# MDIL-SNU/SevenNet

Measured on AMD Instinct MI355X. Metric: atom-steps/sec (energy+forces), SevenNet-0 100k-atom cell, 1/2/4/8 MI355X, higher is better.
Workload: dtype f32 (storage / accumulate / tensor product; in-kernel W2 products f16x3 = two fp16 terms per operand, three matrix-core products: fp32-rounding class; node linears bf16x6); 1 GPU; sevennet_0 shape (5 interaction layers), 97336-atom periodic diamond-Si cell (a=5.431 A x 23^3, sigma=0.05 A), cutoff 5.0 A, 2725408 directed edges, seeded synthetic weights; atoms=97336, edges=2725408, parallelism=single GPU, fused=auto, terms=4

## Files before the change

### include/snet_hip.h

```cpp
#ifndef SNET_HIP_H
#define SNET_HIP_H

#include <stdint.h>

#ifdef __cplusplus
extern "C" {
#endif

#define SNET_ABI_VERSION 4

int snet_abi_version(void);
const char *snet_last_error(void);
int snet_conv_num_shapes(void);
const char *snet_conv_shape_tag(int i);

typedef struct snet_edge_params {
  float cutoff;
  int32_t n_basis;
  int32_t cutoff_kind;
  int32_t poly_p;
  float cutoff_on;
  int32_t lmax;
  int32_t normalize;
} snet_edge_params;
// ... 32 lines not shown
  int64_t c_off;
  int32_t n_src, d, N, reserved;
} snet_gemm_multi_desc;
int snet_gemm_multi(const snet_gemm_multi_desc *descs_host, int32_t n_desc, float *C, int64_t n_nodes, int64_t c_node_stride,
                    const int32_t *row_idx, const float *table, const int32_t *types, void *stream);
int64_t snet_gemm_split_size(int32_t K, int32_t N);
int snet_gemm_split_pack(const float *B_host, int32_t K, int32_t N, void *packed_host);
typedef struct snet_mlp_plan snet_mlp_plan;
int snet_radial_mlp_plan_create(int32_t nb, int32_t h1, int32_t h2, int32_t wn, const float *W0_host,
                                const float *W1_host, const float *W2_host, int32_t act, float cst, int32_t mode,
                                snet_mlp_plan **plan);
void snet_radial_mlp_plan_destroy(snet_mlp_plan *plan);
int snet_radial_mlp_fwd(const snet_mlp_plan *plan, const float *emb, int64_t n_edges, float *w_out, void *stream);
int snet_radial_mlp_bwd(const snet_mlp_plan *plan, const float *emb, const float *g_w, int64_t n_edges,
                        float *g_emb, void *stream);

int snet_act_fwd(const float *z, float *a, int64_t n, int32_t act, float cst, void *stream);
int snet_act_bwd(const float *z, const float *g_a, float *g_z, int64_t n, int32_t act, float cst, void *stream);

typedef struct snet_conv_plan snet_conv_plan;
int snet_conv_plan_create(const char *tag, snet_conv_plan **plan);
void snet_conv_plan_destroy(snet_conv_plan *plan);
int snet_conv_register_library(const char *path);
int snet_conv_plan_dims(const snet_conv_plan *plan, int32_t *dx, int32_t *dout, int32_t *nsh, int32_t *wn);

int snet_conv_fwd(const snet_conv_plan *plan, const float *x, const float *sh, const float *w, const int32_t *w_row,
                  const int32_t *row_ptr, const int32_t *src, int64_t n_dst, float scale, float *out,
                  void *stream);
#define SNET_FUSED_TERMS_DEFAULT 4
typedef struct snet_fused_plan snet_fused_plan;
int snet_radial_mlp_hidden_fwd(const snet_mlp_plan *plan, const float *emb, int64_t n_edges, float *h2, void *stream);
int snet_radial_mlp_hidden_fwd_layers(const snet_mlp_plan *const *plans, int32_t n_layers, const float *emb, int64_t n_edges,
                                      float *const *h2, void *stream);
int snet_radial_mlp_hidden_bwd(const snet_mlp_plan *plan, const float *emb, const float *g_h2, int64_t n_edges,
                               float *g_emb, void *stream);
int snet_conv_fused_available(const snet_conv_plan *plan);
int snet_fused_plan_create(const snet_conv_plan *plan, const snet_mlp_plan *mlp, int32_t terms, snet_fused_plan **out);
void snet_fused_plan_destroy(snet_fused_plan *plan);
int snet_edge_tiles(const int32_t *row_ptr, int64_t n_dst, int32_t *tile_ptr, int32_t *tile_node, int64_t tile_capacity,
                    int64_t *n_tiles, void *stream);
int snet_edge_tiles_packed(const int32_t *row_ptr, int64_t node_begin, int64_t node_end, int32_t *tile_e0,
                           int32_t *tile_nodes, int64_t tile_capacity, int64_t *n_tiles, void *stream);
int snet_fused_plan_tile_mode(const snet_fused_plan *plan);
int snet_conv_plan_transposed(const snet_conv_plan *plan, char *tag, float *col_scale, int32_t *dead, int32_t dead_capacity,
                              int32_t *n_dead);
int snet_edges_by_source(const int32_t *row_ptr, int64_t n_dst, const int32_t *eperm, const int32_t *w_row, int64_t n_edges,
                         int32_t *center_t, int32_t *w_row_t, void *stream);
int snet_conv_fwd_fused(const snet_fused_plan *plan, const float *x, const float *sh, const float *h2,
                        const int32_t *w_row, const int32_t *row_ptr, const int32_t *src, int64_t n_dst, float scale,
                        float *out, void *stream);
int snet_conv_bwd_fused(const snet_fused_plan *plan, const float *x, const float *sh, const float *dsh,
                        const float *h2, const int32_t *w_row, const int32_t *row_ptr, const int32_t *src,
                        const int32_t *tile_ptr, const int32_t *tile_node, int64_t n_tiles, float scale,
                        const float *g_out, float *g_xe, float *g_h2, const float *emb, float *g_emb, float *g_vec,
                        const float *x_rowmax, const float *g_rowmax, void *stream);
int snet_conv_bwd_fused_sh(const snet_fused_plan *plan, const float *x, const float *sh, const float *h2, const int32_t *w_row,
                           const int32_t *row_ptr, const int32_t *src, const int32_t *tile_ptr, const int32_t *tile_node,
                           int64_t n_tiles, float scale, const float *g_out, float *g_xe, float *g_h2, const float *emb,
                           float *g_emb, float *g_sh, const float *x_rowmax, const float *g_rowmax, void *stream);
int snet_fused_plan_has_mlp_tail(const snet_fused_plan *plan);
int snet_fused_plan_prefers_tangent(const snet_fused_plan *plan);
int snet_edge_embed_tangent(const snet_edge_params *p_host, const float *coeffs_host, const float *edge_vec,
                            const int32_t *edge_of_row, int64_t n_rows, float *demb, void *stream);
int snet_radial_mlp_hidden_fwd_layers_tangent(const snet_mlp_plan *const *plans, int32_t n_layers, const float *emb, const float *demb,
                                              int64_t n_rows, float *const *h2, float *const *h2d, void *stream);
int snet_conv_bwd_fused_tangent(const snet_fused_plan *plan, const float *x, const float *sh, const float *dsh, const float *h2,
// ... 269 lines not shown
```

### sevennet_amd/_lib.py

```python
from __future__ import annotations

import ctypes as C
import os

_HERE = os.path.dirname(os.path.abspath(__file__))
ABI_VERSION = 4
LIB_PATH = os.environ.get('SNET_HIP_LIB') or os.path.join(_HERE, 'libsnet_hip.so')

c_f32p = C.c_void_p
c_i32p = C.c_void_p
c_f64p = C.c_void_p
c_stream = C.c_void_p


class EdgeParams(C.Structure):
    _fields_ = [('cutoff', C.c_float), ('n_basis', C.c_int32), ('cutoff_kind', C.c_int32),
                ('poly_p', C.c_int32), ('cutoff_on', C.c_float), ('lmax', C.c_int32),
                ('normalize', C.c_int32)]


class GemmDesc(C.Structure):
    _fields_ = [('B', C.c_void_p), ('B_split', C.c_void_p), ('a_off', C.c_int64), ('c_off', C.c_int64), ('d', C.c_int32), ('K', C.c_int32),
                ('N', C.c_int32), ('accumulate', C.c_int32)]

# ... 19 lines not shown
    'snet_conv_num_shapes': (C.c_int, []),
    'snet_conv_shape_tag': (C.c_char_p, [C.c_int]),
    'snet_edge_embed_fwd': (C.c_int, [C.POINTER(EdgeParams), C.POINTER(C.c_float), c_f32p, C.c_int64, c_f32p,
                                      c_f32p, c_f32p, c_stream]),
    'snet_edge_embed_bwd': (C.c_int, [C.POINTER(EdgeParams), C.POINTER(C.c_float), c_f32p, C.c_int64, c_f32p,
                                      c_f32p, c_f32p, C.c_int32, c_stream]),
    'snet_radial_mlp_plan_create': (C.c_int, [C.c_int32, C.c_int32, C.c_int32, C.c_int32, C.POINTER(C.c_float),
                                              C.POINTER(C.c_float), C.POINTER(C.c_float), C.c_int32, C.c_float,
                                              C.c_int32, C.POINTER(C.c_void_p)]),
    'snet_radial_mlp_plan_destroy': (None, [C.c_void_p]),
    'snet_radial_mlp_fwd': (C.c_int, [C.c_void_p, c_f32p, C.c_int64, c_f32p, c_stream]),
    'snet_radial_mlp_bwd': (C.c_int, [C.c_void_p, c_f32p, c_f32p, C.c_int64, c_f32p, c_stream]),
    'snet_conv_bwd_edge_vec': (C.c_int, [C.c_void_p, c_f32p, c_f32p, c_f32p, c_f32p, c_i32p, c_i32p, c_i32p, C.c_int64,
                                         C.c_float, c_f32p, c_f32p, c_f32p, c_f32p, c_stream]),
    'snet_gemm': (C.c_int, [c_f32p, c_f32p, c_f32p, C.c_int64, C.c_int32, C.c_int32, C.c_int32, C.c_int64,
                            C.c_int64, C.c_int64, C.c_int64, c_i32p, C.c_int32, c_stream]),
    'snet_gemm_grouped': (C.c_int, [C.POINTER(GemmDesc), C.c_int32, c_f32p, c_f32p, C.c_int64, C.c_int64, C.c_int64,
                                    c_i32p, c_stream]),
    'snet_gemm_multi': (C.c_int, [C.POINTER(GemmMultiDesc), C.c_int32, c_f32p, C.c_int64, C.c_int64, c_i32p, c_f32p, c_i32p,
                                  c_stream]),
    'snet_gemm_split_size': (C.c_int64, [C.c_int32, C.c_int32]),
    'snet_gemm_split_pack': (C.c_int, [C.c_void_p, C.c_int32, C.c_int32, C.c_void_p]),
    'snet_act_fwd': (C.c_int, [c_f32p, c_f32p, C.c_int64, C.c_int32, C.c_float, c_stream]),
    'snet_act_bwd': (C.c_int, [c_f32p, c_f32p, c_f32p, C.c_int64, C.c_int32, C.c_float, c_stream]),
    'snet_conv_plan_create': (C.c_int, [C.c_char_p, C.POINTER(C.c_void_p)]),
    'snet_conv_plan_destroy': (None, [C.c_void_p]),
    'snet_conv_register_library': (C.c_int, [C.c_char_p]),
    'snet_conv_plan_dims': (C.c_int, [C.c_void_p, C.POINTER(C.c_int32), C.POINTER(C.c_int32),
                                      C.POINTER(C.c_int32), C.POINTER(C.c_int32)]),
    'snet_conv_fwd': (C.c_int, [C.c_void_p, c_f32p, c_f32p, c_f32p, c_i32p, c_i32p, c_i32p, C.c_int64, C.c_float,
                                c_f32p, c_stream]),
    'snet_radial_mlp_hidden_fwd': (C.c_int, [C.c_void_p, c_f32p, C.c_int64, c_f32p, c_stream]),
    'snet_radial_mlp_hidden_fwd_layers': (C.c_int, [C.POINTER(C.c_void_p), C.c_int32, c_f32p, C.c_int64, C.POINTER(C.c_void_p), c_stream]),
    'snet_radial_mlp_hidden_bwd': (C.c_int, [C.c_void_p, c_f32p, c_f32p, C.c_int64, c_f32p, c_stream]),
    'snet_conv_fused_available': (C.c_int, [C.c_void_p]),
    'snet_conv_plan_transposed': (C.c_int, [C.c_void_p, C.c_char_p, c_f32p, c_i32p, C.c_int32, C.POINTER(C.c_int32)]),
    'snet_edges_by_source': (C.c_int, [c_i32p, C.c_int64, c_i32p, c_i32p, C.c_int64, c_i32p, c_i32p, c_stream]),
    'snet_fused_plan_create': (C.c_int, [C.c_void_p, C.c_void_p, C.c_int32, C.POINTER(C.c_void_p)]),
    'snet_fused_plan_destroy': (None, [C.c_void_p]),
    'snet_edge_tiles': (C.c_int, [c_i32p, C.c_int64, c_i32p, c_i32p, C.c_int64, C.POINTER(C.c_int64), c_stream]),
    'snet_conv_fwd_fused': (C.c_int, [C.c_void_p, c_f32p, c_f32p, c_f32p, c_i32p, c_i32p, c_i32p, C.c_int64, C.c_float,
                                      c_f32p, c_stream]),
    'snet_conv_bwd_fused': (C.c_int, [C.c_void_p, c_f32p, c_f32p, c_f32p, c_f32p, c_i32p, c_i32p, c_i32p, c_i32p,
                                      c_i32p, C.c_int64, C.c_float, c_f32p, c_f32p, c_f32p, c_f32p, c_f32p, c_f32p, c_f32p, c_f32p,
                                      c_stream]),
    'snet_conv_bwd_fused_sh': (C.c_int, [C.c_void_p, c_f32p, c_f32p, c_f32p, c_i32p, c_i32p, c_i32p, c_i32p,
                                         c_i32p, C.c_int64, C.c_float, c_f32p, c_f32p, c_f32p, c_f32p, c_f32p, c_f32p, c_f32p, c_f32p,
                                         c_stream]),
    'snet_fused_plan_has_mlp_tail': (C.c_int, [C.c_void_p]),
    'snet_fused_plan_prefers_tangent': (C.c_int, [C.c_void_p]),
    'snet_edge_embed_tangent': (C.c_int, [C.POINTER(EdgeParams), C.POINTER(C.c_float), c_f32p, c_i32p, C.c_int64, c_f32p, c_stream]),
    'snet_radial_mlp_hidden_fwd_layers_tangent': (C.c_int, [C.POINTER(C.c_void_p), C.c_int32, c_f32p, c_f32p, C.c_int64,
                                                            C.POINTER(C.c_void_p), C.POINTER(C.c_void_p), c_stream]),
    'snet_conv_bwd_fused_tangent': (C.c_int, [C.c_void_p, c_f32p, c_f32p, c_f32p, c_f32p, c_f32p, c_i32p, c_i32p, c_i32p, c_i32p,
                                              c_i32p, C.c_int64, C.c_float, c_f32p, c_f32p, c_f32p, c_f32p, c_f32p, c_f32p,
                                              c_stream]),
    'snet_model_set_layer0_moments': (C.c_int, [C.c_void_p, C.c_int32]),
    'snet_layer0_plan_create': (C.c_int, [C.c_void_p, C.c_void_p, C.c_void_p, C.c_float, C.c_int32, C.POINTER(C.c_void_p)]),
    'snet_layer0_fold': (C.c_int, [C.c_void_p, C.c_int32, C.c_int32, C.c_void_p, C.c_float, C.c_int32, C.c_int32, C.c_void_p]),
    'snet_layer0_plan_destroy': (None, [C.c_void_p]),
    'snet_layer0_scratch_size': (C.c_int64, [C.c_void_p, C.c_int64]),
    'snet_layer0_conv_bwd': (C.c_int, [C.c_void_p, c_f32p, c_f32p, c_f32p, c_i32p, c_i32p, c_i32p, c_i32p, c_i32p, c_f32p, c_f32p, c_f32p,
                                       C.c_int64, c_f32p, c_f32p, c_stream]),
    'snet_model_set_last_layer_merged': (C.c_int, [C.c_void_p, C.c_int32]),
    'snet_lastlayer_plan_create': (C.c_int, [C.c_void_p, C.c_void_p, C.POINTER(C.c_void_p)]),
    'snet_lastlayer_plan_destroy': (None, [C.c_void_p]),
# ... 198 lines not shown
```

### sevennet_amd/csrc/snet_mlp.hip

```cpp
#include <algorithm>
#include <cmath>
#include <cstring>
#include <initializer_list>
#include <vector>

#include "snet_common.h"
#include "snet_split.h"

namespace {

using namespace snet;
constexpr int H = 64;

__device__ __forceinline__ int krow(int s, int half) { return 32 * (s >> 4) + (s & 3) + 8 * ((s & 15) >> 2) + 4 * half; }

__device__ __forceinline__ void hidden_forward(const float *__restrict__ emb, int64_t e_lane, bool e_ok, int nb,
                                               const float *__restrict__ W0, const float *W1s, int act, float cst,
                                               int lane, f32x16 (&z1)[2], f32x16 (&a1)[2], f32x16 (&z2)[2]) {
  const int half = lane >> 5, li = lane & 31;
  z1[0] = zero16();
  z1[1] = zero16();
  for (int s = 0; 2 * s < nb; ++s) {
    const int k = 2 * s + half;
    const float b = (e_ok && k < nb) ? emb[e_lane * nb + k] : 0.f;
// ... 328 lines not shown
    if (more) {
#pragma unroll
      for (int i = 0; i < 3; ++i) st[i] = W2B[(int64_t)(c + 1) * W2B_TILE_U4 + tid + 256 * i];
    }
    f32x16 acc = zero16();
#pragma unroll
    for (int q = 0; q < 4; ++q) {
      bf16x8 b[3];
#pragma unroll
      for (int t = 0; t < 3; ++t) b[t] = as_bf16x8(slab[buf][(q * 3 + t) * 64 + lane]);
      acc = mfma6(a2[q], b, acc);
    }
    const int ch = 32 * c + li;
    if (wave_ok && ch < wn) {
#pragma unroll
      for (int r = 0; r < 16; ++r) {
        const int64_t e = e0 + (r & 3) + 8 * (r >> 2) + 4 * half;
        if (e < E) w_out[e * wn + ch] = acc[r];
      }
    }
    if (more) {
#pragma unroll
      for (int i = 0; i < 3; ++i) slab[buf ^ 1][tid + 256 * i] = st[i];
    }
    __syncthreads();
    buf ^= 1;
  }
}

constexpr int MAX_HIDDEN_LAYERS = 8;
struct HiddenLayers {
  const float *W0[MAX_HIDDEN_LAYERS];
  const u32x4 *W1A[MAX_HIDDEN_LAYERS];
  float *h2[MAX_HIDDEN_LAYERS];
  float *h2d[MAX_HIDDEN_LAYERS];
  float cst[MAX_HIDDEN_LAYERS];
  int act[MAX_HIDDEN_LAYERS];
  int n;
};

template <int ACT, int NB>
__global__ __launch_bounds__(256, 2) void radial_mlp_hidden_layers_kernel(const float *__restrict__ emb, int64_t E, int nb,
                                                                       HiddenLayers P) {
  const int tid = threadIdx.x;
  const int lane = tid & 63, wave = __builtin_amdgcn_readfirstlane(tid >> 6);
  const int half = lane >> 5, li = lane & 31;
  const int64_t e_lane = ((int64_t)blockIdx.x * 4 + wave) * 32 + li;
  const bool e_ok = e_lane < E;
  for (int l = 0; l < P.n; ++l) {
    const int act = P.act[l];
    const float cst = P.cst[l];
    f32x16 z1[2], z2[2];
    hidden_forward_split<ACT, NB>(emb, e_ok ? e_lane : 0, e_ok, nb, P.W0[l], P.W1A[l], act, cst, lane, z1, z2);
    if (!e_ok) continue;
    float *__restrict__ h2 = P.h2[l];
#pragma unroll
    for (int t = 0; t < 2; ++t)
#pragma unroll
      for (int g = 0; g < 4; ++g) {
        f32x4 v;
#pragma unroll
        for (int i = 0; i < 4; ++i) v[i] = act_sel<ACT>(z2[t][4 * g + i], act) * cst;
        *reinterpret_cast<f32x4 *>(h2 + e_lane * H + 32 * t + 8 * g + 4 * half) = v;
      }
  }
}

template <int ACT>
__device__ __forceinline__ void act_pair_sel(float z, int act, float &f, float &g) {
  if constexpr (ACT >= 0) snet::act_pair_radial(z, ACT, f, g);
  else snet::act_pair_radial(z, act, f, g);
}

template <int ACT, int NB>
__global__ __launch_bounds__(256, 2) void radial_mlp_hidden_layers_tangent_kernel(const float *__restrict__ emb,
                                                                               const float *__restrict__ demb, int64_t E, int nb,
                                                                               HiddenLayers P) {
  const int tid = threadIdx.x;
  const int lane = tid & 63, wave = __builtin_amdgcn_readfirstlane(tid >> 6);
  const int half = lane >> 5, li = lane & 31;
  const int64_t e_raw = ((int64_t)blockIdx.x * 4 + wave) * 32 + li;
  const bool e_ok = e_raw < E;
  const int64_t e_lane = e_ok ? e_raw : 0;
  for (int l = 0; l < P.n; ++l) {
    const int act = P.act[l];
    const float cst = P.cst[l];
    const float *__restrict__ W0 = P.W0[l];
    const u32x4 *__restrict__ W1A = P.W1A[l];
    f32x16 z1[2], z1d[2], z2[2], z2d[2];
#pragma unroll
    for (int t = 0; t < 2; ++t) z1[t] = z1d[t] = z2[t] = z2d[t] = zero16();
    auto l1_step = [&](int s, int n_basis) {
      const int k = 2 * s + half;
      const float b = (e_ok && k < n_basis) ? emb[e_lane * n_basis + k] : 0.f;
      const float bd = (e_ok && k < n_basis) ? demb[e_lane * n_basis + k] : 0.f;
#pragma unroll
      for (int t = 0; t < 2; ++t) {
        const float a = (k < n_basis) ? W0[k * H + 32 * t + li] : 0.f;
        z1[t] = __builtin_amdgcn_mfma_f32_32x32x2f32(a, b, z1[t], 0, 0, 0);
        z1d[t] = __builtin_amdgcn_mfma_f32_32x32x2f32(a, bd, z1d[t], 0, 0, 0);
      }
    };
    if constexpr (NB > 0) {
#pragma unroll
      for (int s = 0; 2 * s < NB; ++s) l1_step(s, NB);
    } else {
      for (int s = 0; 2 * s < nb; ++s) l1_step(s, nb);
    }
#pragma unroll
    for (int q = 0; q < 4; ++q) {
      float v[8], vd[8];
#pragma unroll
      for (int i = 0; i < 8; ++i) {
        float f, g;
        act_pair_sel<ACT>(z1[q >> 1][8 * (q & 1) + i], act, f, g);
        v[i] = f * cst;
        vd[i] = g * cst * z1d[q >> 1][8 * (q & 1) + i];
      }
      const Split3 b = split8(v), bd = split8(vd);
#pragma unroll
      for (int to = 0; to < 2; ++to) {
        bf16x8 a[3];
        load_frag3(W1A, to * 4 + q, lane, a);
        z2[to] = mfma6(a, b, z2[to]);
        z2d[to] = mfma6(a, bd, z2d[to]);
      }
    }
    if (!e_ok) continue;
    float *__restrict__ h2 = P.h2[l];
    float *__restrict__ h2d = P.h2d[l];
#pragma unroll
    for (int t = 0; t < 2; ++t)
#pragma unroll
      for (int g = 0; g < 4; ++g) {
        f32x4 v, vd;
#pragma unroll
        for (int i = 0; i < 4; ++i) {
          float f, d;
          act_pair_sel<ACT>(z2[t][4 * g + i], act, f, d);
          v[i] = f * cst;
          vd[i] = d * cst * z2d[t][4 * g + i];
        }
        *reinterpret_cast<f32x4 *>(h2 + e_lane * H + 32 * t + 8 * g + 4 * half) = v;
        *reinterpret_cast<f32x4 *>(h2d + e_lane * H + 32 * t + 8 * g + 4 * half) = vd;
      }
  }
}

#ifndef SNET_MLP_BWD_OCC
#define SNET_MLP_BWD_OCC 3
#endif
#ifndef SNET_MLP_BWD_WAVES
#define SNET_MLP_BWD_WAVES 4
#endif
constexpr int GS_STRIDE = 36;
constexpr int GS_TILE = 32 * GS_STRIDE;
constexpr int SLAB_U4 = 2 * 2 * 3 * 64;

__global__ __launch_bounds__(64 * SNET_MLP_BWD_WAVES, SNET_MLP_BWD_OCC) void radial_mlp_bwd_split_kernel(
    const float *__restrict__ emb, const float *__restrict__ g_w, int64_t E, int nb, int wn,
    const float *__restrict__ W0, const u32x4 *__restrict__ W1A, const u32x4 *__restrict__ W2A,
    const u32x4 *__restrict__ W1A2, const u32x4 *__restrict__ W0A, int act, float cst, float *__restrict__ g_emb) {
  constexpr int NWV = SNET_MLP_BWD_WAVES, NTH = 64 * NWV, NSL = (768 + NTH - 1) / NTH;
  __shared__ float gws[NWV * GS_TILE];
  __shared__ u32x4 slab[2][SLAB_U4];
  const int tid = threadIdx.x;
  const int lane = tid & 63, wave = __builtin_amdgcn_readfirstlane(tid >> 6);
  const int half = lane >> 5, li = lane & 31;
  const int64_t e0 = ((int64_t)blockIdx.x * NWV + wave) * 32;
  const bool wave_ok = e0 < E;
  const int64_t e_lane = e0 + li;
  const bool e_ok = wave_ok && e_lane < E;
  float *tile = gws + wave * GS_TILE;
  const bool vec_ok = (wn & 3) == 0;
  const int srow = lane >> 3, scol = 4 * (lane & 7);
  const int n_chunks = (wn + CH - 1) / CH;

  f32x4 st_g[2][4];
  u32x4 st_w[2][NSL];
// ... 147 lines not shown
      ga1[to] = mfma6(a, b, ga1[to]);
    }
  }
  f32x16 ge = zero16();
#pragma unroll
  for (int q = 0; q < 4; ++q) {
    float v[8];
#pragma unroll
    for (int i = 0; i < 8; ++i) {
      const int r = 8 * (q & 1) + i;
      v[i] = ga1[q >> 1][r] * cst * snet::act_grad(z1[q >> 1][r], act);
    }
    const Split3 b = split8(v);
    bf16x8 a[3];
    load_frag3(W0A, q, lane, a);
    ge = mfma6(a, b, ge);
  }
  if (e_ok) {
#pragma unroll
    for (int r = 0; r < 16; ++r) {
      const int k0 = (r & 3) + 8 * (r >> 2) + 4 * half;
      if (k0 < nb) g_emb[e_lane * nb + k0] += ge[r];
    }
  }
}

}

struct snet_mlp_plan {
  int nb, wn, act, mode;
  float cst;
  float *W0 = nullptr, *W1 = nullptr, *W2 = nullptr, *W2T = nullptr;
  u32x4 *W1A = nullptr, *W2B = nullptr, *W2A = nullptr, *W1A2 = nullptr, *W0A = nullptr;
  std::vector<float> w2_host;
  std::vector<float> w0_host, w1_host;
};

namespace {

inline uint16_t bf16_rne(float v) {
  uint32_t u;
  memcpy(&u, &v, 4);
  u += 0x7fffu + ((u >> 16) & 1u);
  return (uint16_t)(u >> 16);
}
inline float bf16_f(uint16_t h) {
  const uint32_t u = (uint32_t)h << 16;
  float f;
  memcpy(&f, &u, 4);
  return f;
}
inline void split3(float x, uint16_t (&o)[3]) {
  o[0] = bf16_rne(x);
  const float r1 = x - bf16_f(o[0]);
  o[1] = bf16_rne(r1);
  o[2] = bf16_rne(r1 - bf16_f(o[1]));
}
inline int kmap(int q, int half, int i8) {
  const int r = 8 * (q & 1) + i8;
  return 32 * (q >> 1) + (r & 3) + 8 * (r >> 2) + 4 * half;
}
template <class F>
std::vector<uint16_t> pack_frags(int n_frag, F value) {
  std::vector<uint16_t> out((size_t)n_frag * 3 * 64 * 8);
  for (int f = 0; f < n_frag; ++f)
    for (int lane = 0; lane < 64; ++lane)
      for (int i = 0; i < 8; ++i) {
        uint16_t s[3];
        split3(value(f, lane, i), s);
        for (int t = 0; t < 3; ++t) out[(((size_t)f * 3 + t) * 64 + lane) * 8 + i] = s[t];
      }
  return out;
}
template <class T>
int upload(const std::vector<T> &h, void **dev) {
  if (hipMalloc(dev, h.size() * sizeof(T)) != hipSuccess) return 1;
  return hipMemcpy(*dev, h.data(), h.size() * sizeof(T), hipMemcpyHostToDevice) != hipSuccess;
}

}

extern "C" int snet_radial_mlp_plan_create(int32_t nb, int32_t h1, int32_t h2, int32_t wn, const float *W0_host,
                                           const float *W1_host, const float *W2_host, int32_t act, float cst,
                                           int32_t mode, snet_mlp_plan **plan) {
  SNET_REQUIRE(plan != nullptr && W0_host && W1_host && W2_host, "snet_radial_mlp_plan_create: null argument");
  SNET_REQUIRE(h1 == H && h2 == H, "snet_radial_mlp_plan_create: fused kernels need hidden widths [64, 64]");
  SNET_REQUIRE(nb >= 1 && nb <= 32 && wn >= 1, "snet_radial_mlp_plan_create: need 1 <= n_basis <= 32, wn >= 1");
  SNET_REQUIRE(act >= 0 && act < snet::N_ACT, "snet_radial_mlp_plan_create: unknown activation");
  SNET_REQUIRE(mode == 0 || mode == 1, "snet_radial_mlp_plan_create: mode 0 (fp32 MFMA) or 1 (bf16 x6 split)");
  auto *p = new snet_mlp_plan;
  p->nb = nb; p->wn = wn; p->act = act; p->mode = mode; p->cst = cst;
  const std::vector<float> w0(W0_host, W0_host + (size_t)nb * H), w1(W1_host, W1_host + (size_t)H * H),
      w2(W2_host, W2_host + (size_t)H * wn);
  int bad = upload(w0, (void **)&p->W0);
  if (mode == 0) {
    std::vector<float> w2t((size_t)wn * H);
    for (int k = 0; k < H; ++k)
      for (int c = 0; c < wn; ++c) w2t[(size_t)c * H + k] = w2[(size_t)k * wn + c];
    bad |= upload(w1, (void **)&p->W1) | upload(w2, (void **)&p->W2) | upload(w2t, (void **)&p->W2T);
  } else {
    const int n_tiles = (wn + 31) / 32, n_chunks = (wn + CH - 1) / CH;
    bad |= upload(pack_frags(8, [&](int f, int lane, int i) {
                    const int to = f >> 2, q = f & 3;
                    return w1[(size_t)kmap(q, lane >> 5, i) * H + 32 * to + (lane & 31)];
                  }), (void **)&p->W1A);
    bad |= upload(pack_frags(n_tiles * 4, [&](int f, int lane, int i) {
                    const int c = f >> 2, q = f & 3, ch = 32 * c + (lane & 31);
                    return ch < wn ? w2[(size_t)kmap(q, lane >> 5, i) * wn + ch] : 0.f;
                  }), (void **)&p->W2B);
    bad |= upload(pack_frags(n_chunks * 4, [&](int f, int lane, int i) {
                    const int t = f & 1, s = (f >> 1) & 1, ck = f >> 2;
                    const int ch = ck * CH + 16 * s + 8 * (lane >> 5) + i;
                    return ch < wn ? w2[(size_t)(32 * t + (lane & 31)) * wn + ch] : 0.f;
                  }), (void **)&p->W2A);
    bad |= upload(pack_frags(8, [&](int f, int lane, int i) {
                    const int to = f >> 2, q = f & 3;
                    return w1[(size_t)(32 * to + (lane & 31)) * H + kmap(q, lane >> 5, i)];
                  }), (void **)&p->W1A2);
    bad |= upload(pack_frags(4, [&](int f, int lane, int i) {
                    const int k0 = lane & 31;
                    return k0 < nb ? w0[(size_t)k0 * H + kmap(f, lane >> 5, i)] : 0.f;
                  }), (void **)&p->W0A);
  }
  p->w2_host = w2;
  p->w0_host = w0;
  p->w1_host = w1;
  if (bad) {
    snet::set_error("snet_radial_mlp_plan_create: device allocation / upload failed");
    delete p;
    return 1;
  }
  *plan = p;
  return 0;
}

extern "C" void snet_radial_mlp_plan_destroy(snet_mlp_plan *p) {
  if (!p) return;
  for (void *d : {(void *)p->W0, (void *)p->W1, (void *)p->W2, (void *)p->W2T, (void *)p->W1A, (void *)p->W2B,
                  (void *)p->W2A, (void *)p->W1A2, (void *)p->W0A})
    if (d) (void)hipFree(d);
  delete p;
}

extern "C" int snet_radial_mlp_fwd(const snet_mlp_plan *p, const float *emb, int64_t E, float *w_out, void *stream) {
  SNET_REQUIRE(p != nullptr, "snet_radial_mlp_fwd: null plan");
  if (E <= 0) return 0;
  const int64_t grid = (E + 127) / 128;
  SNET_REQUIRE(grid < (1ll << 31), "snet_radial_mlp_fwd: too many edges");
  hipStream_t st = static_cast<hipStream_t>(stream);
  if (p->mode == 0)
    radial_mlp_fwd_kernel<<<(unsigned)grid, 256, 0, st>>>(emb, E, p->nb, p->wn, p->W0, p->W1, p->W2, p->act, p->cst,
                                                          w_out);
  else
    radial_mlp_fwd_split_kernel<<<(unsigned)grid, 256, 0, st>>>(emb, E, p->nb, p->wn, p->W0, p->W1A, p->W2B, p->act,
                                                                p->cst, w_out);
  SNET_CHECK_LAUNCH("snet_radial_mlp_fwd");
  return 0;
}

extern "C" int snet_radial_mlp_hidden_fwd_layers(const snet_mlp_plan *const *plans, int32_t n_layers, const float *emb, int64_t E,
                                                 float *const *h2, void *stream) {
  SNET_REQUIRE(plans != nullptr && h2 != nullptr, "snet_radial_mlp_hidden_fwd_layers: null argument");
  SNET_REQUIRE(n_layers >= 1 && n_layers <= MAX_HIDDEN_LAYERS, "snet_radial_mlp_hidden_fwd_layers: 1 .. 8 layers per call");
  HiddenLayers P{};
  P.n = n_layers;
  bool silu = true;
  for (int l = 0; l < n_layers; ++l) {
    const snet_mlp_plan *p = plans[l];
    SNET_REQUIRE(p != nullptr, "snet_radial_mlp_hidden_fwd_layers: null plan");
    SNET_REQUIRE(E <= 0 || h2[l] != nullptr, "snet_radial_mlp_hidden_fwd_layers: null output");
    SNET_REQUIRE(p->mode == 1, "snet_radial_mlp_hidden_fwd_layers: split-precision plans only (mode 1)");
    SNET_REQUIRE(p->nb == plans[0]->nb, "snet_radial_mlp_hidden_fwd_layers: the layers must share the edge embedding (same n_basis)");
    P.W0[l] = p->W0; P.W1A[l] = p->W1A; P.h2[l] = h2[l]; P.cst[l] = p->cst; P.act[l] = p->act;
    silu = silu && p->act == 0;
  }
  if (E <= 0) return 0;
  const int64_t grid = (E + 127) / 128;
  SNET_REQUIRE(grid < (1ll << 31), "snet_radial_mlp_hidden_fwd_layers: too many edges");
  hipStream_t st = static_cast<hipStream_t>(stream);
  const int nb = plans[0]->nb;
  if (silu && nb == 8) radial_mlp_hidden_layers_kernel<0, 8><<<(unsigned)grid, 256, 0, st>>>(emb, E, nb, P);
  else if (silu) radial_mlp_hidden_layers_kernel<0, 0><<<(unsigned)grid, 256, 0, st>>>(emb, E, nb, P);
  else radial_mlp_hidden_layers_kernel<-1, 0><<<(unsigned)grid, 256, 0, st>>>(emb, E, nb, P);
  SNET_CHECK_LAUNCH("snet_radial_mlp_hidden_fwd_layers");
  return 0;
}

extern "C" int snet_radial_mlp_hidden_fwd_layers_tangent(const snet_mlp_plan *const *plans, int32_t n_layers, const float *emb,
                                                         const float *demb, int64_t E, float *const *h2, float *const *h2d, void *stream) {
  SNET_REQUIRE(plans != nullptr && h2 != nullptr && h2d != nullptr, "snet_radial_mlp_hidden_fwd_layers_tangent: null argument");
  SNET_REQUIRE(n_layers >= 1 && n_layers <= MAX_HIDDEN_LAYERS, "snet_radial_mlp_hidden_fwd_layers_tangent: 1 .. 8 layers per call");
  HiddenLayers P{};
  P.n = n_layers;
  bool silu = true;
  for (int l = 0; l < n_layers; ++l) {
    const snet_mlp_plan *p = plans[l];
    SNET_REQUIRE(p != nullptr, "snet_radial_mlp_hidden_fwd_layers_tangent: null plan");
    SNET_REQUIRE(E <= 0 || (h2[l] != nullptr && h2d[l] != nullptr), "snet_radial_mlp_hidden_fwd_layers_tangent: null output");
    SNET_REQUIRE(p->mode == 1, "snet_radial_mlp_hidden_fwd_layers_tangent: split-precision plans only (mode 1)");
    SNET_REQUIRE(p->nb == plans[0]->nb, "snet_radial_mlp_hidden_fwd_layers_tangent: the layers must share the edge embedding (same n_basis)");
    P.W0[l] = p->W0; P.W1A[l] = p->W1A; P.h2[l] = h2[l]; P.h2d[l] = h2d[l]; P.cst[l] = p->cst; P.act[l] = p->act;
    silu = silu && p->act == 0;
  }
  if (E <= 0) return 0;
  SNET_REQUIRE(emb != nullptr && demb != nullptr, "snet_radial_mlp_hidden_fwd_layers_tangent: null input");
  const int64_t grid = (E + 127) / 128;
  SNET_REQUIRE(grid < (1ll << 31), "snet_radial_mlp_hidden_fwd_layers_tangent: too many edges");
  hipStream_t st = static_cast<hipStream_t>(stream);
  const int nb = plans[0]->nb;
  if (silu && nb == 8) radial_mlp_hidden_layers_tangent_kernel<0, 8><<<(unsigned)grid, 256, 0, st>>>(emb, demb, E, nb, P);
  else if (silu) radial_mlp_hidden_layers_tangent_kernel<0, 0><<<(unsigned)grid, 256, 0, st>>>(emb, demb, E, nb, P);
  else radial_mlp_hidden_layers_tangent_kernel<-1, 0><<<(unsigned)grid, 256, 0, st>>>(emb, demb, E, nb, P);
  SNET_CHECK_LAUNCH("snet_radial_mlp_hidden_fwd_layers_tangent");
  return 0;
}

extern "C" int snet_radial_mlp_hidden_fwd(const snet_mlp_plan *p, const float *emb, int64_t E, float *h2, void *stream) {
  SNET_REQUIRE(p != nullptr, "snet_radial_mlp_hidden_fwd: null plan");
  return snet_radial_mlp_hidden_fwd_layers(&p, 1, emb, E, &h2, stream);
}

namespace snet {
int mlp_plan_wn(const snet_mlp_plan *plan) { return plan ? plan->wn : 0; }
const float *mlp_plan_w2_host(const snet_mlp_plan *plan) {
  return (plan && !plan->w2_host.empty()) ? plan->w2_host.data() : nullptr;
}

MlpHidden mlp_plan_hidden(const snet_mlp_plan *plan) {
  MlpHidden h{nullptr, nullptr, 0, 0, 0.f};
  if (plan && plan->mode == 1 && !plan->w0_host.empty())
    h = MlpHidden{plan->w0_host.data(), plan->w1_host.data(), plan->nb, plan->act, plan->cst};
  return h;
}
uint16_t f16_rne(float f) {
  uint32_t u;
  std::memcpy(&u, &f, 4);
  const uint16_t sign = (uint16_t)((u >> 16) & 0x8000u);
  const uint32_t a = u & 0x7fffffffu;
  if (a >= 0x7f800000u) return sign | (a > 0x7f800000u ? 0x7e00u : 0x7c00u);
  if (a >= 0x477ff000u) return sign | 0x7c00u;
  if (a < 0x33000001u) return sign;
  if (a < 0x38800000u) {
    const int shift = 126 - (int)(a >> 23);
    const uint32_t m = (a & 0x7fffffu) | 0x800000u;
    const uint32_t q = m >> shift, rem = m & ((1u << shift) - 1), half = 1u << (shift - 1);
    return sign | (uint16_t)(q + ((rem > half || (rem == half && (q & 1))) ? 1 : 0));
  }
  const uint32_t r = a + 0xfffu + ((a >> 13) & 1);
  return sign | (uint16_t)((r - 0x38000000u) >> 13);
}
float f16_f(uint16_t h) {
  const uint32_t sign = (uint32_t)(h & 0x8000u) << 16, e = (h >> 10) & 31, m = h & 0x3ffu;
// ... 126 lines not shown
```

Before: 2.857 million atom-steps/s.

## Stage hidden MLP outputs through LDS tiles and keep L1 inputs in registers

Merges the plain and tangent hidden-layer kernels into one templated body. The body loads the edge embedding once, prefetches the next layer's W0 into registers, and applies activations over whole accumulator tiles. Output rows of h2/h2d are staged through a per-wave swizzled LDS tile so global stores are full contiguous 256-byte rows instead of strided 16-byte pieces. An optional scaled two-term f16 matrix-core path for W1 is added behind a compile flag that is off by default. The cost is extra LDS and wave barriers, plus possible register pressure from holding the L1 operands.

```diff
diff --git a/include/snet_hip.h b/include/snet_hip.h
--- a/include/snet_hip.h
+++ b/include/snet_hip.h
@@ -88,6 +88,7 @@
 int snet_radial_mlp_hidden_fwd(const snet_mlp_plan *plan, const float *emb, int64_t n_edges, float *h2, void *stream);
 int snet_radial_mlp_hidden_fwd_layers(const snet_mlp_plan *const *plans, int32_t n_layers, const float *emb, int64_t n_edges,
                                       float *const *h2, void *stream);
+int snet_radial_mlp_pack_w1_f16(const float *W1_host, uint16_t *frags, int32_t *exp_out);
 int snet_radial_mlp_hidden_bwd(const snet_mlp_plan *plan, const float *emb, const float *g_h2, int64_t n_edges,
                                float *g_emb, void *stream);
 int snet_conv_fused_available(const snet_conv_plan *plan);
diff --git a/sevennet_amd/_lib.py b/sevennet_amd/_lib.py
--- a/sevennet_amd/_lib.py
+++ b/sevennet_amd/_lib.py
@@ -75,6 +75,7 @@
                                 c_f32p, c_stream]),
     'snet_radial_mlp_hidden_fwd': (C.c_int, [C.c_void_p, c_f32p, C.c_int64, c_f32p, c_stream]),
     'snet_radial_mlp_hidden_fwd_layers': (C.c_int, [C.POINTER(C.c_void_p), C.c_int32, c_f32p, C.c_int64, C.POINTER(C.c_void_p), c_stream]),
+    'snet_radial_mlp_pack_w1_f16': (C.c_int, [C.POINTER(C.c_float), C.c_void_p, C.POINTER(C.c_int32)]),
     'snet_radial_mlp_hidden_bwd': (C.c_int, [C.c_void_p, c_f32p, c_f32p, C.c_int64, c_f32p, c_stream]),
     'snet_conv_fused_available': (C.c_int, [C.c_void_p]),
     'snet_conv_plan_transposed': (C.c_int, [C.c_void_p, C.c_char_p, c_f32p, c_i32p, C.c_int32, C.POINTER(C.c_int32)]),
diff --git a/sevennet_amd/csrc/snet_mlp.hip b/sevennet_amd/csrc/snet_mlp.hip
--- a/sevennet_amd/csrc/snet_mlp.hip
+++ b/sevennet_amd/csrc/snet_mlp.hip
@@ -384,39 +384,195 @@
 struct HiddenLayers {
   const float *W0[MAX_HIDDEN_LAYERS];
   const u32x4 *W1A[MAX_HIDDEN_LAYERS];
+  const u32x4 *W1H[MAX_HIDDEN_LAYERS];
   float *h2[MAX_HIDDEN_LAYERS];
   float *h2d[MAX_HIDDEN_LAYERS];
   float cst[MAX_HIDDEN_LAYERS];
   int act[MAX_HIDDEN_LAYERS];
+  int w1_exp[MAX_HIDDEN_LAYERS];
   int n;
 };
 
-template <int ACT, int NB>
-__global__ __launch_bounds__(256, 2) void radial_mlp_hidden_layers_kernel(const float *__restrict__ emb, int64_t E, int nb,
-                                                                       HiddenLayers P) {
-  const int tid = threadIdx.x;
-  const int lane = tid & 63, wave = __builtin_amdgcn_readfirstlane(tid >> 6);
+#ifndef SNET_HIDDEN_F16
+#define SNET_HIDDEN_F16 0
+#endif
+#ifndef SNET_HIDDEN_OCC
+#define SNET_HIDDEN_OCC 2
+#endif
+
+__device__ __forceinline__ f32x16 mfma32_f16(bf16x8 a, bf16x8 b, f32x16 acc) {
+  return __builtin_amdgcn_mfma_f32_32x32x16_f16(__builtin_bit_cast(f16x8, a), __builtin_bit_cast(f16x8, b), acc, 0, 0, 0);
+}
+
+__device__ __forceinline__ int tile_scale_exp(const f32x16 (&a)[2]) {
+  float m = 0.f;
+#pragma unroll
+  for (int t = 0; t < 2; ++t)
+#pragma unroll
+    for (int r = 0; r < 16; ++r) m = fmaxf(m, fabsf(a[t][r]));
+  return min(60, F16_TOP - bound_exp(wave_max(m)));
+}
+
+template <int ACT, bool TANGENT>
+__device__ __forceinline__ void hidden_l2(const f32x16 (&a)[2], const f32x16 (&ad)[2], const u32x4 *__restrict__ W1A,
+                                          const u32x4 *__restrict__ W1H, int w1_exp, int lane, f32x16 (&z2)[2], f32x16 (&z2d)[2]) {
+#pragma unroll
+  for (int t = 0; t < 2; ++t) z2[t] = z2d[t] = zero16();
+  if constexpr (ACT >= 0 && SNET_HIDDEN_F16) {
+    u32x4 w[2][2][2];
+    auto load_w = [&](int q) {
+#pragma unroll
+      for (int to = 0; to < 2; ++to)
+#pragma unroll
+        for (int term = 0; term < 2; ++term) w[q & 1][to][term] = W1H[((to * 4 + q) * 2 + term) * 64 + lane];
+    };
+    load_w(0);
+    const int k = tile_scale_exp(a);
+    int kd = 0;
+    if constexpr (TANGENT) kd = tile_scale_exp(ad);
+    const float up = pow2f(k), upd = pow2f(kd);
+#pragma unroll
+    for (int q = 0; q < 4; ++q) {
+      if (q + 1 < 4) {
+        load_w(q + 1);
+        __builtin_amdgcn_sched_barrier(0);
+      }
+      float v[8], vd[8];
+#pragma unroll
+      for (int i = 0; i < 8; ++i) {
+        v[i] = a[q >> 1][8 * (q & 1) + i] * up;
+        if constexpr (TANGENT) vd[i] = ad[q >> 1][8 * (q & 1) + i] * upd;
+      }
+      const SplitN<2> b = splitn8<2, true>(v);
+      SplitN<2> bd;
+      if constexpr (TANGENT) bd = splitn8<2, true>(vd);
+#pragma unroll
+      for (int to = 0; to < 2; ++to) {
+        const bf16x8 w_hi = as_bf16x8(w[q & 1][to][0]), w_lo = as_bf16x8(w[q & 1][to][1]);
+        z2[to] = mfma32_f16(w_hi, b.t[1], z2[to]);
+        z2[to] = mfma32_f16(w_lo, b.t[0], z2[to]);
+        z2[to] = mfma32_f16(w_hi, b.t[0], z2[to]);
+        if constexpr (TANGENT) {
+          z2d[to] = mfma32_f16(w_hi, bd.t[1], z2d[to]);
+          z2d[to] = mfma32_f16(w_lo, bd.t[0], z2d[to]);
+          z2d[to] = mfma32_f16(w_hi, bd.t[0], z2d[to]);
+        }
+      }
+    }
+    const float down = pow2f(-(k + w1_exp)), downd = pow2f(-(kd + w1_exp));
+#pragma unroll
+    for (int t = 0; t < 2; ++t)
+#pragma unroll
+      for (int r = 0; r < 16; ++r) {
+        z2[t][r] *= down;
+        if constexpr (TANGENT) z2d[t][r] *= downd;
+      }
+  } else {
+#pragma unroll
+    for (int q = 0; q < 4; ++q) {
+      float v[8], vd[8];
+#pragma unroll
+      for (int i = 0; i < 8; ++i) {
+        v[i] = a[q >> 1][8 * (q & 1) + i];
+        if constexpr (TANGENT) vd[i] = ad[q >> 1][8 * (q & 1) + i];
+      }
+      const Split3 b = split8(v);
+      Split3 bd;
+      if constexpr (TANGENT) bd = split8(vd);
+#pragma unroll
+      for (int to = 0; to < 2; ++to) {
+        bf16x8 w[3];
+        load_frag3(W1A, to * 4 + q, lane, w);
+        z2[to] = mfma6(w, b, z2[to]);
+        if constexpr (TANGENT) z2d[to] = mfma6(w, bd, z2d[to]);
+      }
+    }
+  }
+}
+
+constexpr int HT_FLOATS = 32 * H;
+__device__ __forceinline__ void tile_put(float *tile, int li, int half, int t, int g, f32x4 v) {
+  const int c = 8 * t + 2 * g + half;
+  *reinterpret_cast<f32x4 *>(tile + li * H + 4 * (c ^ (li & 15))) = v;
+}
+__device__ __forceinline__ void tile_store_rows(const float *tile, int lane, float *__restrict__ out, int64_t e0, int64_t E) {
+  __builtin_amdgcn_fence(__ATOMIC_ACQ_REL, "wavefront");
+  __builtin_amdgcn_wave_barrier();
+  const int c = lane & 15;
+#pragma unroll
+  for (int j = 0; j < 8; ++j) {
+    const int row = 4 * j + (lane >> 4);
+    const f32x4 v = *reinterpret_cast<const f32x4 *>(tile + row * H + 4 * (c ^ (row & 15)));
+    if (e0 + row < E) *reinterpret_cast<f32x4 *>(out + (e0 + row) * H + 4 * c) = v;
+  }
+  __builtin_amdgcn_fence(__ATOMIC_ACQ_REL, "wavefront");
+  __builtin_amdgcn_wave_barrier();
+}
+
+template <int NB, bool TANGENT>
+__device__ __forceinline__ void hidden_l1(const float *__restrict__ emb, const float *__restrict__ demb, int64_t e_lane, bool e_ok, int nb,
+                                          const float *__restrict__ W0, int lane, f32x16 (&z1)[2], f32x16 (&z1d)[2]) {
   const int half = lane >> 5, li = lane & 31;
-  const int64_t e_lane = ((int64_t)blockIdx.x * 4 + wave) * 32 + li;
-  const bool e_ok = e_lane < E;
-  for (int l = 0; l < P.n; ++l) {
-    const int act = P.act[l];
-    const float cst = P.cst[l];
-    f32x16 z1[2], z2[2];
-    hidden_forward_split<ACT, NB>(emb, e_ok ? e_lane : 0, e_ok, nb, P.W0[l], P.W1A[l], act, cst, lane, z1, z2);
-    if (!e_ok) continue;
-    float *__restrict__ h2 = P.h2[l];
-#pragma unroll
-    for (int t = 0; t < 2; ++t)
-#pragma unroll
-      for (int g = 0; g < 4; ++g) {
-        f32x4 v;
-#pragma unroll
-        for (int i = 0; i < 4; ++i) v[i] = act_sel<ACT>(z2[t][4 * g + i], act) * cst;
-        *reinterpret_cast<f32x4 *>(h2 + e_lane * H + 32 * t + 8 * g + 4 * half) = v;
-      }
-  }
-}
+#pragma unroll
+  for (int t = 0; t < 2; ++t) z1[t] = z1d[t] = zero16();
+  auto l1_step = [&](int s, int n_basis) {
+    const int k = 2 * s + half;
+    const float b = (e_ok && k < n_basis) ? emb[e_lane * n_basis + k] : 0.f;
+    float bd = 0.f;
+    if constexpr (TANGENT) bd = (e_ok && k < n_basis) ? demb[e_lane * n_basis + k] : 0.f;
+#pragma unroll
+    for (int t = 0; t < 2; ++t) {
+      const float a = (k < n_basis) ? W0[k * H + 32 * t + li] : 0.f;
+      z1[t] = __builtin_amdgcn_mfma_f32_32x32x2f32(a, b, z1[t], 0, 0, 0);
+      if constexpr (TANGENT) z1d[t] = __builtin_amdgcn_mfma_f32_32x32x2f32(a, bd, z1d[t], 0, 0, 0);
+    }
+  };
+  static_assert(NB == 0, "the compile-time basis count goes through L1Regs");
+  for (int s = 0; 2 * s < nb; ++s) l1_step(s, nb);
+}
+
+template <int NB, bool TANGENT>
+struct L1Regs {
+  static constexpr int S = (NB + 1) / 2 > 0 ? (NB + 1) / 2 : 1;
+  float b[S], bd[S], a[S][2];
+  __device__ __forceinline__ void load_rows(const float *__restrict__ emb, const float *__restrict__ demb, int64_t e_lane, bool e_ok, int lane) {
+    const int half = lane >> 5;
+#pragma unroll
+    for (int s = 0; s < S; ++s) {
+      const int k = 2 * s + half, kc = k < NB ? k : NB - 1;
+      const float v = emb[e_lane * NB + kc];
+      b[s] = (e_ok && k < NB) ? v : 0.f;
+      bd[s] = 0.f;
+      if constexpr (TANGENT) {
+        const float vd = demb[e_lane * NB + kc];
+        bd[s] = (e_ok && k < NB) ? vd : 0.f;
+      }
+    }
+  }
+  __device__ __forceinline__ void load_w0(const float *__restrict__ W0, int lane) {
+    const int half = lane >> 5, li = lane & 31;
+#pragma unroll
+    for (int s = 0; s < S; ++s) {
+      const int k = 2 * s + half, kc = k < NB ? k : NB - 1;
+#pragma unroll
+      for (int t = 0; t < 2; ++t) {
+        const float v = W0[kc * H + 32 * t + li];
+        a[s][t] = k < NB ? v : 0.f;
+      }
+    }
+  }
+  __device__ __forceinline__ void run(f32x16 (&z1)[2], f32x16 (&z1d)[2]) const {
+#pragma unroll
+    for (int t = 0; t < 2; ++t) z1[t] = z1d[t] = zero16();
+#pragma unroll
+    for (int s = 0; s < S; ++s)
+#pragma unroll
+      for (int t = 0; t < 2; ++t) {
+        z1[t] = __builtin_amdgcn_mfma_f32_32x32x2f32(a[s][t], b[s], z1[t], 0, 0, 0);
+        if constexpr (TANGENT) z1d[t] = __builtin_amdgcn_mfma_f32_32x32x2f32(a[s][t], bd[s], z1d[t], 0, 0, 0);
+      }
+  }
+};
 
 template <int ACT>
 __device__ __forceinline__ void act_pair_sel(float z, int act, float &f, float &g) {
@@ -424,79 +580,95 @@
   else snet::act_pair_radial(z, act, f, g);
 }
 
-template <int ACT, int NB>
-__global__ __launch_bounds__(256, 2) void radial_mlp_hidden_layers_tangent_kernel(const float *__restrict__ emb,
-                                                                               const float *__restrict__ demb, int64_t E, int nb,
-                                                                               HiddenLayers P) {
+template <int ACT, int NB, bool TANGENT>
+__device__ __forceinline__ void hidden_layers_body(const float *__restrict__ emb, const float *__restrict__ demb, int64_t E, int nb,
+                                                   const HiddenLayers &P, float *tiles) {
   const int tid = threadIdx.x;
   const int lane = tid & 63, wave = __builtin_amdgcn_readfirstlane(tid >> 6);
   const int half = lane >> 5, li = lane & 31;
-  const int64_t e_raw = ((int64_t)blockIdx.x * 4 + wave) * 32 + li;
-  const bool e_ok = e_raw < E;
-  const int64_t e_lane = e_ok ? e_raw : 0;
+  const int64_t e0 = ((int64_t)blockIdx.x * 4 + wave) * 32;
+  if (e0 >= E) return;
+  const bool e_ok = e0 + li < E;
+  const int64_t e_lane = e_ok ? e0 + li : 0;
+  float *tile = tiles + wave * HT_FLOATS;
+  L1Regs<NB, TANGENT> l1;
+  if constexpr (NB > 0) {
+    l1.load_rows(emb, demb, e_lane, e_ok, lane);
+    l1.load_w0(P.W0[0], lane);
+  }
   for (int l = 0; l < P.n; ++l) {
     const int act = P.act[l];
     const float cst = P.cst[l];
-    const float *__restrict__ W0 = P.W0[l];
-    const u32x4 *__restrict__ W1A = P.W1A[l];
     f32x16 z1[2], z1d[2], z2[2], z2d[2];
-#pragma unroll
-    for (int t = 0; t < 2; ++t) z1[t] = z1d[t] = z2[t] = z2d[t] = zero16();
-    auto l1_step = [&](int s, int n_basis) {
-      const int k = 2 * s + half;
-      const float b = (e_ok && k < n_basis) ? emb[e_lane * n_basis + k] : 0.f;
-      const float bd = (e_ok && k < n_basis) ? demb[e_lane * n_basis + k] : 0.f;
-#pragma unroll
-      for (int t = 0; t < 2; ++t) {
-        const float a = (k < n_basis) ? W0[k * H + 32 * t + li] : 0.f;
-        z1[t] = __builtin_amdgcn_mfma_f32_32x32x2f32(a, b, z1[t], 0, 0, 0);
-        z1d[t] = __builtin_amdgcn_mfma_f32_32x32x2f32(a, bd, z1d[t], 0, 0, 0);
-      }
-    };
     if constexpr (NB > 0) {
-#pragma unroll
-      for (int s = 0; 2 * s < NB; ++s) l1_step(s, NB);
+      l1.run(z1, z1d);
+      if (l + 1 < P.n) l1.load_w0(P.W0[l + 1], lane);
     } else {
-      for (int s = 0; 2 * s < nb; ++s) l1_step(s, nb);
-    }
-#pragma unroll
-    for (int q = 0; q < 4; ++q) {
-      float v[8], vd[8];
-#pragma unroll
-      for (int i = 0; i < 8; ++i) {
-        float f, g;
-        act_pair_sel<ACT>(z1[q >> 1][8 * (q & 1) + i], act, f, g);
-        v[i] = f * cst;
-        vd[i] = g * cst * z1d[q >> 1][8 * (q & 1) + i];
-      }
-      const Split3 b = split8(v), bd = split8(vd);
-#pragma unroll
-      for (int to = 0; to < 2; ++to) {
-        bf16x8 a[3];
-        load_frag3(W1A, to * 4 + q, lane, a);
-        z2[to] = mfma6(a, b, z2[to]);
-        z2d[to] = mfma6(a, bd, z2d[to]);
-      }
-    }
-    if (!e_ok) continue;
-    float *__restrict__ h2 = P.h2[l];
-    float *__restrict__ h2d = P.h2d[l];
+      hidden_l1<NB, TANGENT>(emb, demb, e_lane, e_ok, nb, P.W0[l], lane, z1, z1d);
+    }
+    if constexpr (TANGENT) {
+#pragma unroll
+      for (int t = 0; t < 2; ++t)
+#pragma unroll
+        for (int r = 0; r < 16; ++r) {
+          float f, g;
+          act_pair_sel<ACT>(z1[t][r], act, f, g);
+          z1[t][r] = f * cst;
+          z1d[t][r] = g * cst * z1d[t][r];
+        }
+    } else {
+#pragma unroll
+      for (int t = 0; t < 2; ++t)
+#pragma unroll
+        for (int r = 0; r < 16; ++r) z1[t][r] = act_sel<ACT>(z1[t][r], act) * cst;
+    }
+    hidden_l2<ACT, TANGENT>(z1, z1d, P.W1A[l], P.W1H[l], P.w1_exp[l], lane, z2, z2d);
+    if constexpr (TANGENT) {
+#pragma unroll
+      for (int t = 0; t < 2; ++t)
+#pragma unroll
+        for (int r = 0; r < 16; ++r) {
+          float f, d;
+          act_pair_sel<ACT>(z2[t][r], act, f, d);
+          z2[t][r] = f * cst;
+          z2d[t][r] = d * cst * z2d[t][r];
+        }
+    } else {
+#pragma unroll
+      for (int t = 0; t < 2; ++t)
+#pragma unroll
+        for (int r = 0; r < 16; ++r) z2[t][r] = act_sel<ACT>(z2[t][r], act) * cst;
+    }
 #pragma unroll
     for (int t = 0; t < 2; ++t)
 #pragma unroll
-      for (int g = 0; g < 4; ++g) {
-        f32x4 v, vd;
-#pragma unroll
-        for (int i = 0; i < 4; ++i) {
-          float f, d;
-          act_pair_sel<ACT>(z2[t][4 * g + i], act, f, d);
-          v[i] = f * cst;
-          vd[i] = d * cst * z2d[t][4 * g + i];
-        }
-        *reinterpret_cast<f32x4 *>(h2 + e_lane * H + 32 * t + 8 * g + 4 * half) = v;
-        *reinterpret_cast<f32x4 *>(h2d + e_lane * H + 32 * t + 8 * g + 4 * half) = vd;
-      }
-  }
+      for (int g = 0; g < 4; ++g)
+        tile_put(tile, li, half, t, g, f32x4{z2[t][4 * g], z2[t][4 * g + 1], z2[t][4 * g + 2], z2[t][4 * g + 3]});
+    tile_store_rows(tile, lane, P.h2[l], e0, E);
+    if constexpr (TANGENT) {
+#pragma unroll
+      for (int t = 0; t < 2; ++t)
+#pragma unroll
+        for (int g = 0; g < 4; ++g)
+          tile_put(tile, li, half, t, g, f32x4{z2d[t][4 * g], z2d[t][4 * g + 1], z2d[t][4 * g + 2], z2d[t][4 * g + 3]});
+      tile_store_rows(tile, lane, P.h2d[l], e0, E);
+    }
+  }
+}
+
+template <int ACT, int NB>
+__global__ __launch_bounds__(256, SNET_HIDDEN_OCC) void radial_mlp_hidden_layers_kernel(const float *__restrict__ emb, int64_t E, int nb,
+                                                                                      HiddenLayers P) {
+  __shared__ __attribute__((aligned(16))) float tiles[4 * HT_FLOATS];
+  hidden_layers_body<ACT, NB, false>(emb, nullptr, E, nb, P, tiles);
+}
+
+template <int ACT, int NB>
+__global__ __launch_bounds__(256, SNET_HIDDEN_OCC) void radial_mlp_hidden_layers_tangent_kernel(const float *__restrict__ emb,
+                                                                                              const float *__restrict__ demb, int64_t E,
+                                                                                              int nb, HiddenLayers P) {
+  __shared__ __attribute__((aligned(16))) float tiles[4 * HT_FLOATS];
+  hidden_layers_body<ACT, NB, true>(emb, demb, E, nb, P, tiles);
 }
 
 #ifndef SNET_MLP_BWD_OCC
@@ -710,6 +882,8 @@
   float cst;
   float *W0 = nullptr, *W1 = nullptr, *W2 = nullptr, *W2T = nullptr;
   u32x4 *W1A = nullptr, *W2B = nullptr, *W2A = nullptr, *W1A2 = nullptr, *W0A = nullptr;
+  u32x4 *W1H = nullptr;
+  int w1_exp = 0;
   std::vector<float> w2_host;
   std::vector<float> w0_host, w1_host;
 };
@@ -747,6 +921,20 @@
         uint16_t s[3];
         split3(value(f, lane, i), s);
         for (int t = 0; t < 3; ++t) out[(((size_t)f * 3 + t) * 64 + lane) * 8 + i] = s[t];
+      }
+  return out;
+}
+std::vector<uint16_t> pack_w1_f16(const float *w1, int &exp) {
+  exp = snet::f16_scale_exp(w1, (size_t)H * H);
+  std::vector<uint16_t> out((size_t)8 * 2 * 64 * 8);
+  for (int f = 0; f < 8; ++f)
+    for (int lane = 0; lane < 64; ++lane)
+      for (int i = 0; i < 8; ++i) {
+        const int to = f >> 2, q = f & 3;
+        const float x = std::ldexp(w1[(size_t)kmap(q, lane >> 5, i) * H + 32 * to + (lane & 31)], exp);
+        const uint16_t hi = snet::f16_rne(x), lo = snet::f16_rne(x - snet::f16_f(hi));
+        out[(((size_t)f * 2 + 0) * 64 + lane) * 8 + i] = hi;
+        out[(((size_t)f * 2 + 1) * 64 + lane) * 8 + i] = lo;
       }
   return out;
 }
@@ -782,6 +970,7 @@
                     const int to = f >> 2, q = f & 3;
                     return w1[(size_t)kmap(q, lane >> 5, i) * H + 32 * to + (lane & 31)];
                   }), (void **)&p->W1A);
+    bad |= upload(pack_w1_f16(w1.data(), p->w1_exp), (void **)&p->W1H);
     bad |= upload(pack_frags(n_tiles * 4, [&](int f, int lane, int i) {
                     const int c = f >> 2, q = f & 3, ch = 32 * c + (lane & 31);
                     return ch < wn ? w2[(size_t)kmap(q, lane >> 5, i) * wn + ch] : 0.f;
@@ -815,7 +1004,7 @@
 extern "C" void snet_radial_mlp_plan_destroy(snet_mlp_plan *p) {
   if (!p) return;
   for (void *d : {(void *)p->W0, (void *)p->W1, (void *)p->W2, (void *)p->W2T, (void *)p->W1A, (void *)p->W2B,
-                  (void *)p->W2A, (void *)p->W1A2, (void *)p->W0A})
+                  (void *)p->W2A, (void *)p->W1A2, (void *)p->W0A, (void *)p->W1H})
     if (d) (void)hipFree(d);
   delete p;
 }
@@ -849,7 +1038,7 @@
     SNET_REQUIRE(E <= 0 || h2[l] != nullptr, "snet_radial_mlp_hidden_fwd_layers: null output");
     SNET_REQUIRE(p->mode == 1, "snet_radial_mlp_hidden_fwd_layers: split-precision plans only (mode 1)");
     SNET_REQUIRE(p->nb == plans[0]->nb, "snet_radial_mlp_hidden_fwd_layers: the layers must share the edge embedding (same n_basis)");
-    P.W0[l] = p->W0; P.W1A[l] = p->W1A; P.h2[l] = h2[l]; P.cst[l] = p->cst; P.act[l] = p->act;
+    P.W0[l] = p->W0; P.W1A[l] = p->W1A; P.W1H[l] = p->W1H; P.w1_exp[l] = p->w1_exp; P.h2[l] = h2[l]; P.cst[l] = p->cst; P.act[l] = p->act;
     silu = silu && p->act == 0;
   }
   if (E <= 0) return 0;
@@ -877,7 +1066,8 @@
     SNET_REQUIRE(E <= 0 || (h2[l] != nullptr && h2d[l] != nullptr), "snet_radial_mlp_hidden_fwd_layers_tangent: null output");
     SNET_REQUIRE(p->mode == 1, "snet_radial_mlp_hidden_fwd_layers_tangent: split-precision plans only (mode 1)");
     SNET_REQUIRE(p->nb == plans[0]->nb, "snet_radial_mlp_hidden_fwd_layers_tangent: the layers must share the edge embedding (same n_basis)");
-    P.W0[l] = p->W0; P.W1A[l] = p->W1A; P.h2[l] = h2[l]; P.h2d[l] = h2d[l]; P.cst[l] = p->cst; P.act[l] = p->act;
+    P.W0[l] = p->W0; P.W1A[l] = p->W1A; P.W1H[l] = p->W1H; P.w1_exp[l] = p->w1_exp; P.h2[l] = h2[l]; P.h2d[l] = h2d[l]; P.cst[l] = p->cst;
+    P.act[l] = p->act;
     silu = silu && p->act == 0;
   }
   if (E <= 0) return 0;
@@ -896,6 +1086,15 @@
 extern "C" int snet_radial_mlp_hidden_fwd(const snet_mlp_plan *p, const float *emb, int64_t E, float *h2, void *stream) {
   SNET_REQUIRE(p != nullptr, "snet_radial_mlp_hidden_fwd: null plan");
   return snet_radial_mlp_hidden_fwd_layers(&p, 1, emb, E, &h2, stream);
+}
+
+extern "C" int snet_radial_mlp_pack_w1_f16(const float *W1_host, uint16_t *frags, int32_t *exp_out) {
+  SNET_REQUIRE(W1_host != nullptr && frags != nullptr && exp_out != nullptr, "snet_radial_mlp_pack_w1_f16: null argument");
+  int e = 0;
+  const std::vector<uint16_t> out = pack_w1_f16(W1_host, e);
+  std::memcpy(frags, out.data(), out.size() * sizeof(uint16_t));
+  *exp_out = e;
+  return 0;
 }
 
 namespace snet {
```

Result: no change. 2.860 million atom-steps/s, median of 5 (+0.1%).
